# marl/l3embedding

Hardware: AMD Instinct MI355X
Metric: AVC training pairs/sec (1s audio + 224x224 frame) (higher is better)
Workload: dtype f32; 1 GPU; full cnn_L3_melspec2 AVC training step (audio+vision+fusion, fwd+bwd+Adam), batch 64 per GPU, global batch 64, fp32, inputs resident in HBM; global_batch=64, parallelism=dp1, fp32_conv=f4x4

## Files before the change

### include/l3hip.h

```cpp
#ifndef L3HIP_H
#define L3HIP_H

#include <stdint.h>

#ifdef __cplusplus
extern "C" {
#endif

#define L3_OK 0
#define L3_EINVAL (-1)
#define L3_EHIP (-2)
#define L3_ENOMEM (-3)
#define L3_ESTATE (-4)
#define L3_ECOMM (-5)

#define L3_MODEL_CNN_L3_ORIG 0
#define L3_MODEL_TINY_L3 1
#define L3_MODEL_CNN_L3_KAPREDBINPUTBN 2
#define L3_MODEL_CNN_L3_MELSPEC1 3
#define L3_MODEL_CNN_L3_MELSPEC2 4

typedef struct l3_engine l3_engine;

#define L3_DTYPE_F32 0
// ... 178 lines not shown
                           float *mean, float *var, int n, int h, int wd, int cin, int cout, int kh, int kw, int same,
                           int stat_mode);
int l3_op_conv2d_dgrad_bn_bwd(int device, int dtype, const float *dy, const float *w, const float *bn_x, const float *gamma,
                              const float *beta, const float *mean, const float *var, float *dx, float *part, int *nblk,
                              float *dgamma, float *dbeta, int n, int h, int wd, int cin, int cout, int kh, int kw, int same,
                              int relu, int64_t bn_rows);
int l3_op_first_block_bwd(int device, int form, int relu, const float *x, const float *gamma_in, const float *beta_in, const float *w,
                          const float *y, const float *gamma2, const float *beta2, const float *dA, float *mean_in, float *var_in,
                          float *xaug, float *mean2, float *var2, float *scale2, float *shift2, float *dgamma2, float *dbeta2,
                          float *coeffs, float *dY, float *gaug, float *dw, float *dbias, float *dgamma_in, float *dbeta_in, int n,
                          int h, int wd, int c, int cout);
int l3_op_first_conv_grads(int device, const float *gaug, const float *w, const float *gamma, const float *beta, float *dw,
                           float *dgamma, float *dbeta, float *dbias, int taps, int c, int co);
int l3_op_bn_relu_pool2_fwd_xwin(int device, const float *x, const float *gamma, const float *beta, float *p, float *mean,
                                 float *var, float *xwin, int n, int h, int wd, int c, int same, int relu_mode, int x_bf16);
int l3_op_preprocess(int device, const uint8_t *video_u8, int64_t nv, float *video,
                     const int16_t *audio_i16, int64_t na, float *audio);
int l3_op_augment_video(int device, const uint8_t *u8, int n, int h, int w, const l3_augment_params *params,
                        uint8_t *out_u8, float *out_f32);
int l3_op_augment_audio(int device, const int16_t *i16, int n, int t, const double *u, int16_t *out_i16, float *out_f32,
                        double *gains);

typedef struct l3_mlp l3_mlp;
int l3_mlp_create(int device, int D, int C, int batch, float weight_decay, uint64_t seed, l3_mlp **m);
void l3_mlp_destroy(l3_mlp *m);
int64_t l3_mlp_param_count(const l3_mlp *m);
int l3_mlp_set_data(l3_mlp *m, const float *X_train, const int32_t *y_train, int64_t n_train,
                    const float *X_valid, const int32_t *y_valid, int64_t n_valid);
int l3_mlp_epoch(l3_mlp *m, const int32_t *perm, float lr, int64_t t0, double *stats_out);
int l3_mlp_predict(l3_mlp *m, const float *X, int64_t n, float *probs_out);
// ... 195 lines not shown
```

### l3embedding_amd/_lib.py

```python
import ctypes as C
import os

import numpy as np

from . import _build

MODEL_IDS = {
    'cnn_L3_orig': 0,
    'tiny_L3': 1,
    'cnn_L3_kapredbinputbn': 2,
    'cnn_L3_melspec1': 3,
    'cnn_L3_melspec2': 4,
}

FAMILIES = ('conv_fwd', 'conv_dgrad', 'conv_wgrad', 'elementwise', 'frontend', 'head', 'adam')


DTYPES = {'f32': 0, 'fp32': 0, 'float32': 0, 'bf16': 1}
FP32_CONV = {'f4x4': 0, 'f2x2': 1, 'f2x2_bf16x6': 2}
DP_MOVING = {'replicas': 0, 'rank_local': 1}
OP_DTYPES = dict(DTYPES, bf16_stored=2, bf16_stored_out=3)


class L3Config(C.Structure):
# ... 125 lines not shown
    'l3_op_gather_frames': (C.c_int, [C.c_int, C.c_void_p, C.c_int64, C.c_void_p, C.c_int64, C.c_void_p]),
    'l3_op_image_frames': (C.c_int, [C.c_int, C.c_void_p, C.c_int64, C.c_void_p, C.c_int64, C.c_void_p, C.c_void_p]),
    'l3_op_resample': (C.c_int, [C.c_int, C.c_void_p, C.c_int64, C.c_int64, C.c_int64, C.c_void_p, C.c_int64, C.c_int,
                                 C.c_int64, C.c_int64, C.c_void_p]),
    'l3_op_resample_clips': (C.c_int, [C.c_int, C.c_void_p, C.c_int64, C.c_void_p, C.c_int64, C.c_int64, C.c_void_p, C.c_int64,
                                       C.c_int, C.c_int64, C.c_int, C.c_void_p]),
    'l3_op_bn_stats_from_partials': (C.c_int, [C.c_int, C.c_void_p, C.c_int, C.c_int, C.c_void_p, C.c_int64, C.c_float,
                                               C.c_void_p, C.c_void_p]),
    'l3_op_conv2d_fwd_stats': (C.c_int, [C.c_int, C.c_int] + [C.c_void_p] * 5 + [C.POINTER(C.c_int), C.c_void_p, C.c_void_p] +
                               [C.c_int] * 9),
    'l3_op_conv2d_dgrad_bn_bwd': (C.c_int, [C.c_int, C.c_int] + [C.c_void_p] * 9 + [C.POINTER(C.c_int), C.c_void_p, C.c_void_p] +
                                  [C.c_int] * 9 + [C.c_int64]),
    'l3_op_first_block_bwd': (C.c_int, [C.c_int] * 3 + [C.c_void_p] * 24 + [C.c_int] * 5),
    'l3_op_first_conv_grads': (C.c_int, [C.c_int] + [C.c_void_p] * 8 + [C.c_int] * 3),
    'l3_op_bn_relu_pool2_fwd_xwin': (C.c_int, [C.c_int] + [C.c_void_p] * 7 + [C.c_int] * 7),
    'l3_op_preprocess': (C.c_int, [C.c_int, C.c_void_p, C.c_int64, C.c_void_p, C.c_void_p, C.c_int64, C.c_void_p]),
    'l3_op_augment_video': (C.c_int, [C.c_int, C.c_void_p, C.c_int, C.c_int, C.c_int, C.c_void_p, C.c_void_p, C.c_void_p]),
    'l3_op_augment_audio': (C.c_int, [C.c_int, C.c_void_p, C.c_int, C.c_int, C.c_void_p, C.c_void_p, C.c_void_p, C.c_void_p]),
    'l3_mlp_create': (C.c_int, [C.c_int, C.c_int, C.c_int, C.c_int, C.c_float, C.c_uint64, C.POINTER(C.c_void_p)]),
    'l3_mlp_destroy': (None, [C.c_void_p]),
    'l3_mlp_param_count': (C.c_int64, [C.c_void_p]),
    'l3_mlp_set_data': (C.c_int, [C.c_void_p, C.c_void_p, C.c_void_p, C.c_int64, C.c_void_p, C.c_void_p, C.c_int64]),
    'l3_mlp_epoch': (C.c_int, [C.c_void_p, C.c_void_p, C.c_float, C.c_int64, C.POINTER(C.c_double)]),
    'l3_mlp_predict': (C.c_int, [C.c_void_p, C.c_void_p, C.c_int64, C.c_void_p]),
    'l3_mlp_get_weights': (C.c_int, [C.c_void_p, C.c_void_p, C.c_int64]),
    'l3_mlp_set_weights': (C.c_int, [C.c_void_p, C.c_void_p, C.c_int64]),
    'l3_op_mlp_dense_fwd': (C.c_int, [C.c_int, C.c_void_p, C.c_int64, C.c_void_p, C.c_int, C.c_int, C.c_int, C.c_void_p,
                                      C.c_void_p, C.c_int, C.c_void_p]),
    'l3_op_mlp_dense_bwd_x': (C.c_int, [C.c_int, C.c_void_p, C.c_void_p, C.c_void_p, C.c_int, C.c_int, C.c_int, C.c_void_p]),
    'l3_op_mlp_wgrad': (C.c_int, [C.c_int, C.c_void_p, C.c_int64, C.c_void_p, C.c_int, C.c_int, C.c_int, C.c_void_p,
# ... 706 lines not shown
                                      _ptr(var), n, h, wd, c, int(same), int(relu_mode), flags))
    return p, mean, var


def op_bn_relu_pool2_bwd(x, gamma, beta, dp, same, device=0, relu_mode=1, x_bf16=False, out_bf16=False):
    lib = load()
    x, dp = _f32(x), _f32(dp)
    n, h, wd, c = x.shape
    dx = np.empty_like(x)
    dg, db, dbias = (np.empty((c,), np.float32) for _ in range(3))
    check(lib.l3_op_bn_relu_pool2_bwd(device, _ptr(x), _ptr(_f32(gamma)), _ptr(_f32(beta)), _ptr(dp), _ptr(dx),
                                      _ptr(dg), _ptr(db), _ptr(dbias), n, h, wd, c, int(same), int(relu_mode), int(x_bf16) | (4 if out_bf16 else 0)))
    return dx, dg, db, dbias


def _pool_out(h, p, s, same):
    return -(-h // s) if same else (h - p) // s + 1


def op_maxpool_fwd(x, ph, pw, sh, sw, same, device=0):
    lib = load()
    x = _f32(x)
    n, h, wd, c = x.shape
    y = np.empty((n, _pool_out(h, ph, sh, same), _pool_out(wd, pw, sw, same), c), np.float32)
    check(lib.l3_op_maxpool_fwd(device, _ptr(x), _ptr(y), n, h, wd, c, ph, pw, sh, sw, int(same)))
    return y


def op_maxpool_bwd(x, dy, ph, pw, sh, sw, same, device=0):
    lib = load()
# ... 1147 lines not shown
```

### l3embedding_amd/csrc/bn_fused.hip

```cpp
#include "kernels.h"
#include "device_common.h"

namespace l3 {



__device__ __forceinline__ void store_quad(void* base, int64_t q, f32x4 v, int obf) {
    if (obf) {
        bf16x4 h;
        h[0] = (__bf16)v.x; h[1] = (__bf16)v.y; h[2] = (__bf16)v.z; h[3] = (__bf16)v.w;
        __builtin_nontemporal_store(h, reinterpret_cast<bf16x4*>(base) + q);
    } else {
        __builtin_nontemporal_store(v, reinterpret_cast<f32x4*>(base) + q);
    }
}

template <bool XBF>
__device__ __forceinline__ f32x4 load_quad(const void* base, int64_t q) {
    if constexpr (XBF) {
        const u32x2 r = __builtin_nontemporal_load(reinterpret_cast<const u32x2*>(base) + q);
        return f32x4{__uint_as_float(r.x << 16), __uint_as_float(r.x & 0xffff0000u), __uint_as_float(r.y << 16),
                     __uint_as_float(r.y & 0xffff0000u)};
    } else {
        return __builtin_nontemporal_load(reinterpret_cast<const f32x4*>(base) + q);
// ... 563 lines not shown
    const int nb_a = fast_blocks(work_a);
    float* part2 = dbias ? part : nullptr;
    using ApplyFn = void (*)(const void*, const void*, const f32x4*, const f32x4*, const f32x4*, const f32x4*, const f32x4*, void*,
                             float*, int64_t, Pool2Geom, int, int);
    static const ApplyFn apply_fns[8] = {
        bn_bwd_apply_fast_kernel<false, false, false>, bn_bwd_apply_fast_kernel<false, false, true>,
        bn_bwd_apply_fast_kernel<false, true, false>,  bn_bwd_apply_fast_kernel<false, true, true>,
        bn_bwd_apply_fast_kernel<true, false, false>,  bn_bwd_apply_fast_kernel<true, false, true>,
        bn_bwd_apply_fast_kernel<true, true, false>,   bn_bwd_apply_fast_kernel<true, true, true>};
    hipLaunchKernelGGL(apply_fns[variant], dim3(nb_a), dim3(FB), 0, s, xv, dyv, sc4, sh4, reinterpret_cast<const f32x4*>(cA),
                       reinterpret_cast<const f32x4*>(cB), reinterpret_cast<const f32x4*>(cC), (void*)dx, part2, n4, g, relu,
                       dx_bf16);
    if (dbias) launch_fast_final(SumFinal{dbias}, part, nb_a, C, s);
}

}
```

### l3embedding_amd/csrc/elementwise.hip

```cpp
#include <algorithm>

#include "kernels.h"

namespace l3 {

static constexpr int RED_BLOCK = 256;
static constexpr int RED_MAX_BLOCKS = 1024;
static constexpr int SMALLC_MAX = 16;

static inline int red_blocks(int64_t rows, int C) {
    int rows_per_pass = (C % 4 == 0 && C >= 4 && C <= 1024) ? (RED_BLOCK / (C / 4) > 0 ? RED_BLOCK / (C / 4) : 1) : RED_BLOCK;
    int64_t b = (rows + (int64_t)rows_per_pass * 16 - 1) / ((int64_t)rows_per_pass * 16);
    if (b < 1) b = 1;
    if (b > RED_MAX_BLOCKS) b = RED_MAX_BLOCKS;
    return (int)b;
}

size_t colreduce_scratch_floats(int64_t rows, int C) {
    const size_t a = (size_t)red_blocks(rows, C) * 2 * (size_t)(C < 4 ? 4 : C) + 64;
    const size_t b = bn_fast_ok(C) ? bn_fast_scratch_floats(C) : 0;
    return a > b ? a : b;
}

template <class F>
// ... 510 lines not shown
    int arg[4];
    const size_t base = (size_t)n * P * C + cb * 64 + cq * 4;
    gp_scan(x + base, P, C, pg, best, arg);
    gp_merge(sb, sa, pg, cq, best, arg);
    const gp4 d = *reinterpret_cast<const gp4*>(dy + (size_t)n * out_batch_stride + cb * 64 + cq * 4);
    int am[4];
#pragma unroll
    for (int e = 0; e < 4; ++e) am[e] = sa[0][cq * 4 + e];
    for (int p = pg; p < P; p += 16) {
        gp4 o;
#pragma unroll
        for (int e = 0; e < 4; ++e) o[e] = p == am[e] ? d[e] : 0.f;
        *reinterpret_cast<gp4*>(dx + base + (size_t)p * C) = o;
    }
}
static bool is_global_pool(const PoolGeom& g) {
    return g.Ho == 1 && g.Wo == 1 && g.padT == 0 && g.padL == 0 && g.ph == g.H && g.pw == g.W && g.C % 64 == 0 &&
           g.out_batch_stride % 4 == 0;
}

void maxpool_fwd(const float* x, float* y, const PoolGeom& g, hipStream_t s) {
    if (is_global_pool(g)) {
        hipLaunchKernelGGL(global_maxpool_fwd_kernel, dim3(g.N * (g.C / 64)), dim3(256), 0, s, x, y, g.H * g.W, g.C,
                           (int64_t)g.out_batch_stride);
        return;
    }
    const int64_t total = (int64_t)g.N * g.Ho * g.Wo * g.C;
    hipLaunchKernelGGL(maxpool_fwd_kernel, dim3(ew_blocks(total)), dim3(256), 0, s, x, y, g);
}
__global__ __launch_bounds__(256) void maxpool_bwd_kernel(const float* x, const float* dy, float* dx, PoolGeom g) {
    const int64_t total = (int64_t)g.N * g.Ho * g.Wo * g.C;
// ... 395 lines not shown
```

### l3embedding_amd/csrc/engine.hip

```cpp
#include <hip/hip_runtime.h>
#include "knobs.h"

#include <cmath>
#include <cstdio>
#include <cstdlib>
#include <cstring>
#include <map>
#include <string>
#include <vector>

#include "../../include/l3hip.h"
#include "comm.h"
#include "conv_path.h"
#include "featprep.h"
#include "kernels.h"

namespace {

using namespace l3;

static thread_local std::string g_create_error;

constexpr float BN_EPS = 1e-3f;
constexpr float BN_MOMENTUM = 0.99f;
// ... 29 lines not shown
};

enum FirstWgrad { FW_NONE, FW_AUG, FW_AUG_DEFERRED };
struct ConvPlan {
    ConvStorage st;
    ConvFwdPath fwd;
    int stat_mode = 0;
    FirstWgrad aug = FW_NONE;
    ConvWgradPath wgrad;
    bool colsum = false;
    ConvDgradPath dgrad;
    int bwd_bn = -1;
    double fwd_bytes = 0.0, wg_bytes = 0.0, dg_bytes = 0.0;
};
enum BnStats { BS_PARTIALS, BS_FAST, BS_PLAIN, BS_MOVING };
enum BnBwd { BB_BY_FIRST_CONV, BB_FAST_POOLED, BB_FAST, BB_FAST_DEFERRED, BB_PLAIN };
struct BnPlan {
    BnStats stats = BS_MOVING;
    int stat_blocks = 0;
    BnBwd bwd = BB_PLAIN;
    int bwd_blocks = 0;
    double fwd_bytes = 0.0, bwd_bytes = 0.0;
};

struct Op {
    OpKind kind;
    std::string name;
    int in = 0, out = 0;
    int block = 0, bucket = 0;
    int kh = 0, kw = 0, cout = 0;
    bool same = false;
// ... 6 lines not shown
    bool fused_first = false;
    bool defer_apply = false;
    int bn_defer = -1;
    float *xaug = nullptr, *gaug = nullptr;
    ConvGeom ageom{};
    int bn_follow = -1;
    bool need_dx = true;
    int dy_to_bn = -1;
    float* xwin = nullptr;
    int p_gamma = -1, p_beta = -1, p_mmean = -1, p_mvar = -1;
    bool fused_relu = false;
    bool prerelu = false;
    int fuse_pool = -1;
    int bias_param = -1;
    bool fused_into_bn = false;
    bool bias_by_bn = false;
    float *mean = nullptr, *var = nullptr, *scale = nullptr, *shift = nullptr;
    float *biased_mean = nullptr, *biased_var = nullptr;
    PoolGeom pg{};
    ConvPlan cp{};
    BnPlan bp{};
};

struct Tower {
    std::string prefix;
    std::vector<Tensor> t;
    std::vector<Op> ops;
    int nblocks = 0;
    int emb_conv_op = -1;
    bool training = false;
// ... 507 lines not shown
                tw->ops[i + 1].fused_into_bn = true;
            }
        }
    const int first_wg_fuse = knob_int("L3_FIRST_WG_FUSE", 1);
    if (first_wg_fuse)
        for (Tower* tw : {&e->vis, &e->aud})
            for (auto& cv : tw->ops) {
                if (cv.kind != OP_CONV || cv.in_bn < 0 || cv.bn_follow < 0 || !cv.bias_by_bn) continue;
                Op& bn = tw->ops[cv.bn_follow];
                if (bn.kind == OP_BN && bn.fuse_pool < 0 && !bn.prerelu && bn.in == cv.out && bn_fast_ok(cv.cout) &&
                    conv_first_wgrad_ok(cv.ageom)) {
                    bn.defer_apply = true;
                    cv.bn_defer = cv.bn_follow;
                }
            }
    const int pooled_fuse = knob_int("L3_BNBWD_FUSE_POOLED", 1);
    if (bnbwd_fuse && pooled_fuse)
        for (Tower* tw : {&e->vis, &e->aud})
            for (size_t i = 0; i < tw->ops.size(); ++i) {
                Op& cv = tw->ops[i];
                if (cv.kind != OP_CONV || !cv.need_dx || cv.dy_to_bn >= 0) continue;
                for (size_t j = 0; j < i; ++j) {
                    const Op& bn = tw->ops[j];
                    if (bn.kind == OP_BN && bn.fuse_pool >= 0 && tw->ops[bn.fuse_pool].out == cv.in && (bn.fused_relu != bn.prerelu) &&
                        bn_fast_ok(tw->t[bn.in].C))
                        cv.dy_to_bn = (int)j;
                }
            }
    return L3_OK;
}
// ... 333 lines not shown
                y.alias = true;
                if (op.kind == OP_POOL) op.pg.out_batch_stride = D;
            } else if ((op.kind == OP_BN && op.fuse_pool >= 0) || (op.kind == OP_RELU && op.fused_into_bn)) {
                if (op.kind == OP_BN) {
                    bool wanted = false;
                    for (size_t ci = 0; ci < tw.ops.size(); ++ci)
                        if (tw.ops[ci].kind == OP_CONV && tw.ops[ci].dy_to_bn == (int)oi) wanted = true;
                    const Tensor& pl = tw.t[tw.ops[op.fuse_pool].out];
                    if (wanted && (rc = dev_alloc_t(e, &op.xwin, t_floats(pl, tw.t[op.in].d_bf16)))) return rc;
                }
            } else {
                if ((rc = dev_alloc_t(e, &y.d, t_floats(y, y.d_bf16)))) return rc;
                if ((rc = dev_alloc_t(e, &y.g, t_floats(y, y.g_bf16)))) return rc;
            }
            const Tensor& x = tw.t[op.in];
            if (op.kind == OP_CONV) {
                if ((rc = dev_alloc_t(e, &op.wflip, (size_t)e->params[op.p_kernel].numel))) return rc;
                if (conv_wino_floats(op.geom) && (rc = dev_alloc_t(e, &op.wino_uf, conv_wino_floats(op.geom)))) return rc;
                {
                    const size_t sf = (size_t)conv_wino_stat_blocks_max(op.geom) * 2 * op.geom.Cout;
                    if (sf > stat_max) stat_max = sf;
                    const size_t sb = (size_t)conv_bf16_stat_blocks(op.geom) * 2 * op.geom.Cout;
                    if (e->cfg.dtype == L3_DTYPE_BF16 && sb > stat_max) stat_max = sb;
                    const size_t s1 = (size_t)conv_first_stat_blocks(op.geom) * 2 * op.geom.Cout;
                    if (s1 > stat_max) stat_max = s1;
                    const size_t sd = op.dy_to_bn >= 0 ? (size_t)conv_wino_stat_blocks_max(op.dgeom) * 2 * op.dgeom.Cout : 0;
                    if (sd > stat_max) stat_max = sd;
                    const size_t sdb = op.dy_to_bn >= 0 && e->cfg.dtype == L3_DTYPE_BF16
                                           ? (size_t)conv_bf16_stat_blocks(op.dgeom) * 2 * op.dgeom.Cout : 0;
                    if (sdb > stat_max) stat_max = sdb;
// ... 97 lines not shown
        conv_fwd(e->frames, e->wdft, nullptr, e->spec, g, e->stream);
    }
    {
        ProfScope ps(e, F_FRONTEND, f.n_mels ? 2.0 * B * f.n_frames * (double)f.n_freq * f.n_mels : 0.0);
        spec_to_features(e->spec, e->melw, e->mel_start, e->mel_len, e->mel_off, e->aud.t[0].d, B, f, e->stream, e->dft_nyq);
        if (f.db) db_normalize(e->aud.t[0].d, e->smax, B, e->aud.t[0].batch_stride, e->cfg.db_max_scope, e->stream);
    }
    return L3_OK;
}

static inline double act_bytes(const Tensor& t) { return (double)t.numel() * (t.d_bf16 ? 2.0 : 4.0); }
static inline double grad_bytes(const Tensor& t) { return (double)t.numel() * (t.g_bf16 ? 2.0 : 4.0); }

int plan_tower(l3_engine* e, Tower& tw, bool training, int solo) {
    static const int epi_stats = knob_int("L3_EPILOGUE_STATS", 1);
    const bool bf16 = e->cfg.dtype == L3_DTYPE_BF16;
    tw.training = training;
    auto fits = [&](const Op& cv, int blocks, int C) {
        if ((size_t)blocks * 2 * C <= e->stat_max) return true;
        e->err = cv.name + ": " + std::to_string(blocks) + " partial blocks of " + std::to_string(C) + " channels exceed the statistics scratch (" +
                 std::to_string(e->stat_max) + " floats)";
        return false;
    };
    auto defers = [&](const Op& bn) {
        return training && bn.defer_apply && bn.fuse_pool < 0 && bn_fast_ok(tw.t[bn.in].C) && tw.t[bn.in].d_bf16 == tw.t[bn.out].g_bf16;
    };
    for (auto& op : tw.ops) op.bp = BnPlan{};
    for (auto& op : tw.ops) {
        if (op.kind != OP_CONV) continue;
        op.geom.solo = op.dgeom.solo = solo;
        op.geom.dynamic = op.dgeom.dynamic = e->comm != nullptr ? 1 : 0;
        float* ts = solo ? e->w4_tail : nullptr;
        op.geom.tail_scratch = op.dgeom.tail_scratch = ts;
        op.geom.tail_scratch_bytes = op.dgeom.tail_scratch_bytes = ts ? conv_wino4_tail_scratch_bytes() : 0;

        const Tensor &x = tw.t[op.in], &y = tw.t[op.out];
        const double wbytes = (double)e->params[op.p_kernel].numel * 4.0;
        ConvPlan& p = op.cp = ConvPlan{};
        p.st = ConvStorage{bf16, x.d_bf16, y.d_bf16, y.g_bf16, x.g_bf16};
        p.fwd = conv_resolve_fwd(op.geom, p.st, op.wino_uf != nullptr);
        p.fwd_bytes = act_bytes(x) + act_bytes(y) + wbytes;
        const int nblk = conv_fwd_stat_blocks(p.fwd, op.geom);
// ... 25 lines not shown
    }
    for (auto& op : tw.ops) {
        if (op.kind != OP_BN) continue;
        const Tensor &x = tw.t[op.in], &y = tw.t[op.out];
        const Tensor& out = op.fuse_pool >= 0 ? tw.t[tw.ops[op.fuse_pool].out] : y;
        BnPlan& p = op.bp;
        p.stats = !training ? BS_MOVING : p.stat_blocks > 0 ? BS_PARTIALS : op.prerelu || x.d_bf16 ? BS_FAST : BS_PLAIN;
        p.bwd = training && op.fused_first ? BB_BY_FIRST_CONV : !bn_fast_ok(x.C) ? BB_PLAIN : op.fuse_pool >= 0 ? BB_FAST_POOLED
                : defers(op) ? BB_FAST_DEFERRED : BB_FAST;
        p.fwd_bytes = (!training ? 0.0 : p.stat_blocks > 0 ? (double)p.stat_blocks * 2 * x.C * 4 : act_bytes(x)) + act_bytes(x) + act_bytes(out);
        if (p.bwd == BB_BY_FIRST_CONV) p.fwd_bytes += act_bytes(x) + (double)x.rows() * (&op + 1)->ageom.Cin * 4.0;
        if (op.fuse_pool >= 0 && training && op.xwin != nullptr) p.fwd_bytes += (double)out.numel() * (x.d_bf16 ? 2.0 : 4.0);
        p.bwd_bytes = p.bwd == BB_PLAIN ? 2.0 * (act_bytes(x) + grad_bytes(y)) + grad_bytes(x)
                                        : (p.bwd_blocks > 0 ? (double)p.bwd_blocks * 2 * x.C * 4 : act_bytes(x) + grad_bytes(out)) +
                                              (p.bwd == BB_FAST_DEFERRED ? 0.0 : act_bytes(x) + grad_bytes(out) + grad_bytes(x));
    }
    return L3_OK;
}

void tower_forward(l3_engine* e, Tower& tw) {
    const bool training = tw.training;
    for (auto& op : tw.ops) {
        Tensor& x = tw.t[op.in];
        Tensor& y = tw.t[op.out];
        switch (op.kind) {
            case OP_CONV: {
                const ConvPlan& p = op.cp;
                ConvBufs b;
                b.x = x.d, b.w = e->params[op.p_kernel].d, b.bias = e->params[op.p_bias].d, b.y = y.d;
                b.wprep = op.wflip, b.wino_u = op.wino_uf;
// ... 15 lines not shown
                                               op.scale, op.shift, x.rows(), x.C, BN_EPS, op.prerelu ? 1 : 0, e->stream);
                        break;
                    case BS_FAST:
                        bn_stats_fast(x.d, gamma, beta, op.mean, op.var, op.scale, op.shift, e->red_scratch, x.rows(), x.C, BN_EPS,
                                      op.prerelu ? 1 : 0, e->stream, x.d_bf16 ? 1 : 0);
                        break;
                    case BS_PLAIN:
                        bn_stats(x.d, gamma, beta, op.mean, op.var, op.scale, op.shift, e->red_scratch, x.rows(), x.C, BN_EPS, e->stream);
                        break;
                    case BS_MOVING:
                        bn_scale_shift(gamma, beta, e->params[op.p_mmean].d, e->params[op.p_mvar].d, op.scale, op.shift, x.C, BN_EPS,
                                       e->stream);
                        break;
                }
                if (p.bwd == BB_BY_FIRST_CONV) bn_xhat_ones(x.d, op.mean, op.var, BN_EPS, (&op + 1)->xaug, x.rows(), x.C, e->stream);
                if (op.fuse_pool >= 0) {
                    Tensor& pl = tw.t[tw.ops[op.fuse_pool].out];
                    bn_relu_pool2_fwd(x.d, op.scale, op.shift, pl.d, x.N, x.H, x.W, x.C, pl.H, pl.W, pl.batch_stride,
                                      op.prerelu ? 2 : (op.fused_relu ? 1 : 0), e->stream, pl.d_bf16 ? 1 : 0, x.d_bf16 ? 1 : 0,
                                      training ? (void*)op.xwin : nullptr);
                } else if (y.d_bf16 || x.d_bf16) {
                    bn_apply_fast(x.d, op.scale, op.shift, y.d, x.rows(), x.C, op.fused_relu ? 1 : 0, e->stream, y.d_bf16 ? 1 : 0,
                                  x.d_bf16 ? 1 : 0);
                } else {
                    bn_apply(x.d, op.scale, op.shift, y.d, x.rows(), x.C, op.fused_relu ? 1 : 0, e->stream);
                }
                break;
            }
            case OP_RELU: {
                if (op.fused_into_bn) break;
                ProfScope ps(e, F_ELEMWISE, 0.0);
                ps.bytes(act_bytes(x) + act_bytes(y));
                relu_fwd(x.d, y.d, x.numel(), e->stream);
                break;
            }
            case OP_POOL: {
                if (op.fused_into_bn) break;
                ProfScope ps(e, F_ELEMWISE, 0.0);
                ps.bytes(act_bytes(x) + act_bytes(y));
                maxpool_fwd(x.d, y.d, op.pg, e->stream);
                break;
            }
            default: break;
        }
    }
}

BnBwdFuse bn_bwd_fuse(const Tower& tw, const Op& bn) {
    return BnBwdFuse{bn.fuse_pool >= 0 ? bn.xwin : tw.t[bn.in].d, bn.scale, bn.shift, bn.mean, bn.var, BN_EPS, bn.fused_relu ? 1 : 0};
}

void tower_backward_block(l3_engine* e, Tower& tw, int block) {
    const bool training = tw.training;
    for (int oi = (int)tw.ops.size() - 1; oi >= 0; --oi) {
        Op& op = tw.ops[oi];
        if (op.block != block) continue;
        Tensor& x = tw.t[op.in];
        Tensor& y = tw.t[op.out];
        switch (op.kind) {
            case OP_POOL: {
                if (op.fused_into_bn) break;
                ProfScope ps(e, F_ELEMWISE, 0.0);
                ps.bytes(act_bytes(x) + grad_bytes(y) + grad_bytes(x));
                maxpool_bwd(x.d, y.g, x.g, op.pg, e->stream);
                break;
            }
            case OP_RELU: {
                if (op.fused_into_bn) break;
                ProfScope ps(e, F_ELEMWISE, 0.0);
                ps.bytes(act_bytes(y) + grad_bytes(y) + grad_bytes(x));
                relu_bwd(y.d, y.g, x.g, x.numel(), e->stream);
                break;
            }
            case OP_BN: {
                const BnPlan& p = op.bp;
                if (p.bwd == BB_BY_FIRST_CONV) break;
                ProfScope ps(e, F_ELEMWISE, 0.0);
                ps.bytes(p.bwd_bytes);
                const float* mean = training ? op.mean : e->params[op.p_mmean].d;
                const float* var = training ? op.var : e->params[op.p_mvar].d;
                const float* gamma = e->params[op.p_gamma].d;
                float *dgamma = e->params[op.p_gamma].g, *dbeta = e->params[op.p_beta].g;
                if (p.bwd == BB_PLAIN) {
                    bn_bwd(x.d, y.d, y.g, gamma, mean, var, x.g, dgamma, dbeta, e->red_scratch, x.rows(), x.C, BN_EPS, op.fused_relu ? 1 : 0,
                           training ? 1 : 0, e->stream);
                    break;
                }
                const bool pooled = p.bwd == BB_FAST_POOLED, defer = p.bwd == BB_FAST_DEFERRED;
                const Tensor& dy = pooled ? tw.t[tw.ops[op.fuse_pool].out] : y;
                bn_bwd_fast(x.d, op.scale, op.shift, mean, var, gamma, dy.g, pooled ? 1 : 0, x.N, x.H, x.W, x.C, dy.H, dy.W,
                            pooled ? dy.batch_stride : (int64_t)x.H * x.W * x.C, defer ? nullptr : x.g, dgamma, dbeta,
                            defer ? nullptr : op.bias_param >= 0 ? e->params[op.bias_param].g : nullptr, e->red_scratch, BN_EPS,
                            pooled ? (op.prerelu ? 2 : 1) : (op.fused_relu ? 1 : 0), training ? 1 : 0, e->stream, x.g_bf16 ? 1 : 0,
                            x.d_bf16 ? 1 : 0, dy.g_bf16 ? 1 : 0, p.bwd_blocks > 0 ? e->stat_scratch : nullptr, p.bwd_blocks);
                break;
            }
            case OP_CONV: {
                const ConvPlan& p = op.cp;
                const float* w = e->params[op.p_kernel].d;
                if (p.aug != FW_NONE) {
// ... 1661 lines not shown
```

### l3embedding_amd/csrc/kernels.h

```cpp
#pragma once
#include <hip/hip_runtime.h>
#include <stdint.h>

#include <string>
#include <vector>

#include "host_common.h"

struct l3_clipbank;
struct l3_sample;

namespace l3 {

struct ConvGeom {
    int N, H, W, Cin;
    int Ho, Wo, Cout;
    int KH, KW, padT, padL;
    int f2x2 = 0;
    int solo = 0;
    int dynamic = 0;
    float* tail_scratch = nullptr;
    size_t tail_scratch_bytes = 0;
};
size_t conv_wino4_tail_scratch_bytes();
// ... 99 lines not shown
                   float* shift, float* scratch, int64_t rows, int C, float eps, int prerelu, hipStream_t s, int x_bf16 = 0);
void bn_stats_from_partials(const float* part, int nblk, const float* pivot, const float* gamma, const float* beta,
                            float* mean, float* var, float* scale, float* shift, int64_t rows, int C, float eps,
                            int prerelu, hipStream_t s);
void bn_apply_fast(const float* x, const float* scale, const float* shift, float* y, int64_t rows, int C, int relu,
                   hipStream_t s, int out_bf16 = 0, int x_bf16 = 0);
void bn_relu_pool2_fwd(const float* x, const float* scale, const float* shift, float* p, int N, int H, int W, int C,
                       int Ho, int Wo, int64_t out_batch_stride, int mode, hipStream_t s, int out_bf16 = 0, int x_bf16 = 0,
                       void* xwin = nullptr);
void bn_bwd_fast(const float* x, const float* scale, const float* shift, const float* mean, const float* var,
                 const float* gamma, const float* dy, int pooled, int N, int H, int W, int C, int Ho, int Wo,
                 int64_t dy_batch_stride, float* dx, float* dgamma, float* dbeta, float* dbias, float* scratch,
                 float eps, int relu, int training, hipStream_t s, int dx_bf16 = 0, int x_bf16 = 0, int dy_bf16 = 0,
                 const float* ready_part = nullptr, int ready_blocks = 0);
const float* bn_bwd_fast_coeffs(const float* scratch, int C);

void relu_fwd(const float* x, float* y, int64_t n, hipStream_t s);
void relu_bwd(const float* y, const float* dy, float* dx, int64_t n, hipStream_t s);

struct PoolGeom {
    int N, H, W, C, Ho, Wo, ph, pw, sh, sw, padT, padL;
    int64_t out_batch_stride;
};
void maxpool_fwd(const float* x, float* y, const PoolGeom& g, hipStream_t s);
void maxpool_bwd(const float* x, const float* dy, float* dx, const PoolGeom& g, hipStream_t s);

void preprocess_video(const uint8_t* u8, float* out, int64_t n, hipStream_t s);
void preprocess_audio(const int16_t* pcm, float* out, int64_t n, hipStream_t s);
void labels_onehot(const int32_t* lab, float* out, int64_t n, hipStream_t s);

struct AugmentParams {
    int32_t start_x, start_y, flip, sat_first;
    float saturation, brightness;
};
constexpr int AUG_CROP = 224;
void augment_video(const uint8_t* u8, int N, int H, int W, const AugmentParams* params, uint8_t* out_u8, float* out_f32,
                   hipStream_t s);
void augment_audio(const int16_t* pcm, int N, int T, const double* u, int16_t* out_i16, float* out_f32, double* gains,
// ... 175 lines not shown
```

### l3embedding_amd/csrc/ops.hip

```cpp
#include <hip/hip_runtime.h>

#include <cstring>
#include <string>
#include <vector>

#include "../../include/l3hip.h"
#include "conv_path.h"
#include "kernels.h"
#include "knobs.h"
#include "mlp.h"
#include "vggish.h"

namespace {
using namespace l3;

struct Scope {
    DeviceBufs bufs;
    hipStream_t s = nullptr;
    bool ok = true;
    explicit Scope(int device) : ok(device_ok(device)) {}
    ~Scope() { (void)hipDeviceSynchronize(); }
    template <class T>
    T* alloc(size_t count) {
        T* p = bufs.alloc<T>(count);
// ... 894 lines not shown
    l3_engine* e = nullptr;
    int rc = l3_create(&cfg, 1, &e);
    if (rc) return rc;
    rc = l3_upload_batch(e, nullptr, audio, nullptr);
    if (!rc) rc = l3_step_forward(e, 0);
    int64_t numel = 0;
    if (!rc) rc = l3_activation_numel(e, "audio_model/frontend", &numel);
    if (!rc) rc = l3_get_activation(e, "audio_model/frontend", out, numel);
    l3_destroy(e);
    return rc;
}

}

namespace {
int mlp_op_check(const char* name, int device, bool ptrs_ok, int rows, int K, int N, const int32_t* idx, int64_t n_x) {
    if (!ptrs_ok || rows <= 0 || K <= 0 || N <= 0 || n_x < 0) {
        set_op_error(std::string(name) + ": NULL pointer or non-positive size");
        return L3_EINVAL;
    }
    if (!idx && n_x < rows) {
        set_op_error(std::string(name) + ": fewer rows in x than `rows`");
        return L3_EINVAL;
    }
    for (int i = 0; idx && i < rows; ++i)
        if (idx[i] < 0 || idx[i] >= n_x) {
            set_op_error(std::string(name) + ": idx[" + std::to_string(i) + "] outside [0, n_x)");
            return L3_EINVAL;
        }
    if (!device_ok(device)) {
// ... 487 lines not shown
```

Before: 2049 pairs/s.

## Fuse final BatchNorm+ReLU with global max pool in tower forward and backward

```diff
diff --git a/include/l3hip.h b/include/l3hip.h
--- a/include/l3hip.h
+++ b/include/l3hip.h
@@ -216,6 +216,10 @@
                            float *dgamma, float *dbeta, float *dbias, int taps, int c, int co);
 int l3_op_bn_relu_pool2_fwd_xwin(int device, const float *x, const float *gamma, const float *beta, float *p, float *mean,
                                  float *var, float *xwin, int n, int h, int wd, int c, int same, int relu_mode, int x_bf16);
+int l3_op_bn_relu_gpool_fwd(int device, const float *x, const float *gamma, const float *beta, float *p, int32_t *arg,
+                            float *mean, float *var, int n, int h, int wd, int c);
+int l3_op_bn_relu_gpool_bwd(int device, const float *x, const float *gamma, const float *beta, const float *dp, float *dx,
+                            float *dgamma, float *dbeta, float *dbias, int n, int h, int wd, int c);
 int l3_op_preprocess(int device, const uint8_t *video_u8, int64_t nv, float *video,
                      const int16_t *audio_i16, int64_t na, float *audio);
 int l3_op_augment_video(int device, const uint8_t *u8, int n, int h, int w, const l3_augment_params *params,
diff --git a/l3embedding_amd/_lib.py b/l3embedding_amd/_lib.py
--- a/l3embedding_amd/_lib.py
+++ b/l3embedding_amd/_lib.py
@@ -163,6 +163,8 @@
     'l3_op_first_block_bwd': (C.c_int, [C.c_int] * 3 + [C.c_void_p] * 24 + [C.c_int] * 5),
     'l3_op_first_conv_grads': (C.c_int, [C.c_int] + [C.c_void_p] * 8 + [C.c_int] * 3),
     'l3_op_bn_relu_pool2_fwd_xwin': (C.c_int, [C.c_int] + [C.c_void_p] * 7 + [C.c_int] * 7),
+    'l3_op_bn_relu_gpool_fwd': (C.c_int, [C.c_int] + [C.c_void_p] * 7 + [C.c_int] * 4),
+    'l3_op_bn_relu_gpool_bwd': (C.c_int, [C.c_int] + [C.c_void_p] * 8 + [C.c_int] * 4),
     'l3_op_preprocess': (C.c_int, [C.c_int, C.c_void_p, C.c_int64, C.c_void_p, C.c_void_p, C.c_int64, C.c_void_p]),
     'l3_op_augment_video': (C.c_int, [C.c_int, C.c_void_p, C.c_int, C.c_int, C.c_int, C.c_void_p, C.c_void_p, C.c_void_p]),
     'l3_op_augment_audio': (C.c_int, [C.c_int, C.c_void_p, C.c_int, C.c_int, C.c_void_p, C.c_void_p, C.c_void_p, C.c_void_p]),
@@ -899,6 +901,29 @@
     return dx, dg, db, dbias
 
 
+def op_bn_relu_gpool_fwd(x, gamma, beta, device=0):
+    lib = load()
+    x = _f32(x)
+    n, h, wd, c = x.shape
+    p, arg = np.empty((n, c), np.float32), np.empty((n, c), np.int32)
+    mean, var = np.empty((c,), np.float32), np.empty((c,), np.float32)
+    check(lib.l3_op_bn_relu_gpool_fwd(device, _ptr(x), _ptr(_f32(gamma)), _ptr(_f32(beta)), _ptr(p), _ptr(arg), _ptr(mean), _ptr(var),
+                                      n, h, wd, c))
+    return p, arg, mean, var
+
+
+def op_bn_relu_gpool_bwd(x, gamma, beta, dp, device=0):
+    lib = load()
+    x, dp = _f32(x), _f32(dp)
+    n, h, wd, c = x.shape
+    assert dp.shape == (n, c)
+    dx = np.empty_like(x)
+    dg, db, dbias = (np.empty((c,), np.float32) for _ in range(3))
+    check(lib.l3_op_bn_relu_gpool_bwd(device, _ptr(x), _ptr(_f32(gamma)), _ptr(_f32(beta)), _ptr(dp), _ptr(dx), _ptr(dg), _ptr(db),
+                                      _ptr(dbias), n, h, wd, c))
+    return dx, dg, db, dbias
+
+
 def _pool_out(h, p, s, same):
     return -(-h // s) if same else (h - p) // s + 1
 
diff --git a/l3embedding_amd/csrc/bn_fused.hip b/l3embedding_amd/csrc/bn_fused.hip
--- a/l3embedding_amd/csrc/bn_fused.hip
+++ b/l3embedding_amd/csrc/bn_fused.hip
@@ -601,4 +601,163 @@
     if (dbias) launch_fast_final(SumFinal{dbias}, part, nb_a, C, s);
 }
 
-}
+static constexpr int GP_G = 16;
+static constexpr int GP_U = 8;
+
+bool bn_relu_gpool_ok(int N, int H, int W, int C) {
+    return bn_fast_ok(C) && C % 64 == 0 && N >= 1 && H >= 1 && W >= 1 && (int64_t)H * W < ((int64_t)1 << 30) &&
+           (int64_t)N * (C / 64) < ((int64_t)1 << 31);
+}
+
+__global__ __launch_bounds__(256) void bn_relu_gpool_fwd_kernel(const float* __restrict__ x, const float* __restrict__ scale,
+                                                                const float* __restrict__ shift, float* __restrict__ out,
+                                                                int* __restrict__ arg, int P, int C, int64_t out_batch_stride) {
+    __shared__ float sb[GP_G][64];
+    __shared__ int sa[GP_G][64];
+    const int cb = blockIdx.x % (C / 64), n = blockIdx.x / (C / 64);
+    const int cq = threadIdx.x & 15, pg = threadIdx.x >> 4;
+    const int c0 = cb * 64 + cq * 4;
+    const f32x4 sc = *reinterpret_cast<const f32x4*>(scale + c0), sh = *reinterpret_cast<const f32x4*>(shift + c0);
+    const f32x4* xb = reinterpret_cast<const f32x4*>(x + (size_t)n * P * C + c0);
+    const size_t C4 = (size_t)(C / 4);
+    float best[4];
+    int am[4];
+#pragma unroll
+    for (int e = 0; e < 4; ++e) {
+        best[e] = -INFINITY;
+        am[e] = 0x7fffffff;
+    }
+    for (int p0 = pg; p0 < P; p0 += GP_G * GP_U) {
+        f32x4 v[GP_U];
+#pragma unroll
+        for (int u = 0; u < GP_U; ++u)
+            if (p0 + u * GP_G < P) v[u] = __builtin_nontemporal_load(xb + (size_t)(p0 + u * GP_G) * C4);
+#pragma unroll
+        for (int u = 0; u < GP_U; ++u) {
+            const int p = p0 + u * GP_G;
+            if (p < P) {
+                const f32x4 r = relu4(bn_pre(v[u], sc, sh));
+#pragma unroll
+                for (int e = 0; e < 4; ++e)
+                    if (r[e] > best[e]) {
+                        best[e] = r[e];
+                        am[e] = p;
+                    }
+            }
+        }
+    }
+#pragma unroll
+    for (int e = 0; e < 4; ++e) {
+        sb[pg][cq * 4 + e] = best[e];
+        sa[pg][cq * 4 + e] = am[e];
+    }
+    __syncthreads();
+    if (threadIdx.x < 64) {
+        float b = sb[0][threadIdx.x];
+        int a = sa[0][threadIdx.x];
+        for (int k = 1; k < GP_G; ++k) {
+            const float vb = sb[k][threadIdx.x];
+            const int va = sa[k][threadIdx.x];
+            if (vb > b || (vb == b && va < a)) {
+                b = vb;
+                a = va;
+            }
+        }
+        out[(size_t)n * out_batch_stride + cb * 64 + threadIdx.x] = b;
+        arg[(size_t)n * C + cb * 64 + threadIdx.x] = a;
+    }
+}
+
+void bn_relu_gpool_fwd(const float* x, const float* scale, const float* shift, float* out, int* arg, int N, int H, int W, int C,
+                       int64_t out_batch_stride, hipStream_t s) {
+    hipLaunchKernelGGL(bn_relu_gpool_fwd_kernel, dim3(N * (C / 64)), dim3(256), 0, s, x, scale, shift, out, arg, H * W, C,
+                       out_batch_stride);
+}
+
+__global__ __launch_bounds__(FB) void bn_gpool_bwd_reduce_kernel(const float* __restrict__ x, const float* __restrict__ dp,
+                                                                 const int* __restrict__ arg, const float* __restrict__ scale,
+                                                                 const float* __restrict__ shift, const float* __restrict__ mean,
+                                                                 const float* __restrict__ var, float* __restrict__ part, int N,
+                                                                 int P, int C, int64_t dp_batch_stride, int npb, float eps) {
+    const int n0 = blockIdx.x * npb, n1 = n0 + npb < N ? n0 + npb : N;
+    for (int c = threadIdx.x; c < C; c += FB) {
+        const float sc = scale[c], sh = shift[c], mu = mean[c], rs = rsqrtf(var[c] + eps);
+        float a0 = 0.f, a1 = 0.f;
+        for (int n = n0; n < n1; ++n) {
+            const int a = arg[(size_t)n * C + c];
+            if ((unsigned)a < (unsigned)P) {
+                const float xv = x[((size_t)n * P + a) * C + c];
+                const float d = fmaf(xv, sc, sh) > 0.f ? dp[(size_t)n * dp_batch_stride + c] : 0.f;
+                a0 += d;
+                a1 += d * ((xv - mu) * rs);
+            }
+        }
+        part[((size_t)blockIdx.x * 2 + 0) * C + c] = a0;
+        part[((size_t)blockIdx.x * 2 + 1) * C + c] = a1;
+    }
+}
+
+__global__ __launch_bounds__(FB) void bn_gpool_bwd_apply_kernel(const float* __restrict__ x, const float* __restrict__ dp,
+                                                                const int* __restrict__ arg, const f32x4* scale, const f32x4* shift,
+                                                                const f32x4* cA, const f32x4* cB, const f32x4* cC,
+                                                                float* __restrict__ dx, float* part, int P, int C4,
+                                                                int64_t dp_bs4, int tiles_per_n, int64_t tiles) {
+    constexpr int U = 4, K = 2;
+    const int c4 = (int)threadIdx.x % C4, r = (int)threadIdx.x / C4, rpi = FB / C4;
+    const f32x4 sc = scale[c4], sh = shift[c4], A = cA[c4], B = cB[c4], Cc = cC[c4];
+    f32x4 a0 = {0.f, 0.f, 0.f, 0.f};
+    for (int64_t t = blockIdx.x; t < tiles; t += gridDim.x) {
+        const int n = (int)(t / tiles_per_n);
+        const int pt = (int)(t % tiles_per_n) * (rpi * U * K);
+        const i32x4 am = reinterpret_cast<const i32x4*>(arg)[(int64_t)n * C4 + c4];
+        const f32x4 d = reinterpret_cast<const f32x4*>(dp)[(int64_t)n * dp_bs4 + c4];
+        const int64_t row0 = (int64_t)n * P;
+#pragma unroll
+        for (int k = 0; k < K; ++k) {
+            const int p0 = pt + k * U * rpi + r;
+            f32x4 v[U];
+#pragma unroll
+            for (int u = 0; u < U; ++u)
+                if (p0 + u * rpi < P) v[u] = load_quad<false>(x, (row0 + p0 + u * rpi) * C4 + c4);
+#pragma unroll
+            for (int u = 0; u < U; ++u) {
+                const int p = p0 + u * rpi;
+                if (p < P) {
+                    const f32x4 pre = bn_pre(v[u], sc, sh);
+                    f32x4 dz;
+                    dz.x = p == am.x && pre.x > 0.f ? d.x : 0.f; dz.y = p == am.y && pre.y > 0.f ? d.y : 0.f;
+                    dz.z = p == am.z && pre.z > 0.f ? d.z : 0.f; dz.w = p == am.w && pre.w > 0.f ? d.w : 0.f;
+                    const f32x4 o = A * dz + (B * v[u] + Cc);
+                    store_quad(dx, (row0 + p) * C4 + c4, o, 0);
+                    a0 += o;
+                }
+            }
+        }
+    }
+    if (part != nullptr) block_write_partials(a0, a0, part, C4);
+}
+
+void bn_relu_gpool_bwd(const float* x, const float* scale, const float* shift, const float* mean, const float* var,
+                       const float* gamma, const float* dp, const int* arg, int N, int H, int W, int C, int64_t dp_batch_stride,
+                       float* dx, float* dgamma, float* dbeta, float* dbias, float* scratch, float eps, hipStream_t s) {
+    const int P = H * W, C4 = C / 4;
+    float* part = scratch;
+    float* cA = scratch + (size_t)FAST_MAX_BLOCKS * 2 * C;
+    float* cB = cA + C;
+    float* cC = cB + C;
+    const int npb = (N + FAST_MAX_BLOCKS - 1) / FAST_MAX_BLOCKS;
+    const int nb_r = (N + npb - 1) / npb;
+    hipLaunchKernelGGL(bn_gpool_bwd_reduce_kernel, dim3(nb_r), dim3(FB), 0, s, x, dp, arg, scale, shift, mean, var, part, N, P, C,
+                       dp_batch_stride, npb, eps);
+    launch_fast_final(BwdFinal{gamma, mean, var, dgamma, dbeta, cA, cB, cC, 1.0 / ((double)N * P), eps, 1}, part, nb_r, C, s);
+    const int tile_px = (FB / C4) * 8;
+    const int tiles_per_n = (P + tile_px - 1) / tile_px;
+    const int64_t tiles = (int64_t)N * tiles_per_n;
+    const int nb_a = (int)(tiles < FAST_MAX_BLOCKS ? tiles : FAST_MAX_BLOCKS);
+    hipLaunchKernelGGL(bn_gpool_bwd_apply_kernel, dim3(nb_a), dim3(FB), 0, s, x, dp, arg, reinterpret_cast<const f32x4*>(scale),
+                       reinterpret_cast<const f32x4*>(shift), reinterpret_cast<const f32x4*>(cA), reinterpret_cast<const f32x4*>(cB),
+                       reinterpret_cast<const f32x4*>(cC), dx, dbias ? part : nullptr, P, C4, dp_batch_stride / 4, tiles_per_n, tiles);
+    if (dbias) launch_fast_final(SumFinal{dbias}, part, nb_a, C, s);
+}
+
+}
diff --git a/l3embedding_amd/csrc/elementwise.hip b/l3embedding_amd/csrc/elementwise.hip
--- a/l3embedding_amd/csrc/elementwise.hip
+++ b/l3embedding_amd/csrc/elementwise.hip
@@ -548,7 +548,7 @@
         *reinterpret_cast<gp4*>(dx + base + (size_t)p * C) = o;
     }
 }
-static bool is_global_pool(const PoolGeom& g) {
+bool is_global_pool(const PoolGeom& g) {
     return g.Ho == 1 && g.Wo == 1 && g.padT == 0 && g.padL == 0 && g.ph == g.H && g.pw == g.W && g.C % 64 == 0 &&
            g.out_batch_stride % 4 == 0;
 }
diff --git a/l3embedding_amd/csrc/engine.hip b/l3embedding_amd/csrc/engine.hip
--- a/l3embedding_amd/csrc/engine.hip
+++ b/l3embedding_amd/csrc/engine.hip
@@ -67,7 +67,7 @@
     double fwd_bytes = 0.0, wg_bytes = 0.0, dg_bytes = 0.0;
 };
 enum BnStats { BS_PARTIALS, BS_FAST, BS_PLAIN, BS_MOVING };
-enum BnBwd { BB_BY_FIRST_CONV, BB_FAST_POOLED, BB_FAST, BB_FAST_DEFERRED, BB_PLAIN };
+enum BnBwd { BB_BY_FIRST_CONV, BB_FAST_POOLED, BB_FAST, BB_FAST_DEFERRED, BB_PLAIN, BB_FAST_GPOOL };
 struct BnPlan {
     BnStats stats = BS_MOVING;
     int stat_blocks = 0;
@@ -104,6 +104,9 @@
     int fuse_pool = -1;
     int bias_param = -1;
     bool fused_into_bn = false;
+    int gpool = -1;
+    int* garg = nullptr;
+    bool pass_by_bn = false;
     bool bias_by_bn = false;
     float *mean = nullptr, *var = nullptr, *scale = nullptr, *shift = nullptr;
     float *biased_mean = nullptr, *biased_var = nullptr;
@@ -641,6 +644,16 @@
                     cv.bn_defer = cv.bn_follow;
                 }
             }
+    for (Tower* tw : {&e->vis, &e->aud})
+        if (tw->ops.size() >= 2) {
+            const size_t i = tw->ops.size() - 2;
+            Op& bn = tw->ops[i];
+            const Op& pl = tw->ops[i + 1];
+            const Tensor& x = tw->t[bn.in];
+            if (bn.kind == OP_BN && bn.fused_relu && !bn.prerelu && bn.fuse_pool < 0 && !bn.fused_first && !bn.defer_apply &&
+                pl.kind == OP_POOL && pl.in == bn.out && is_global_pool(pl.pg) && bn_relu_gpool_ok(x.N, x.H, x.W, x.C))
+                bn.gpool = (int)i + 1;
+        }
     const int pooled_fuse = knob_int("L3_BNBWD_FUSE_POOLED", 1);
     if (bnbwd_fuse && pooled_fuse)
         for (Tower* tw : {&e->vis, &e->aud})
@@ -1004,6 +1017,7 @@
                 if ((rc = dev_alloc_t(e, &y.g, t_floats(y, y.g_bf16)))) return rc;
             }
             const Tensor& x = tw.t[op.in];
+            if (op.kind == OP_BN && op.gpool >= 0 && (rc = dev_alloc_t(e, &op.garg, (size_t)x.N * x.C))) return rc;
             if (op.kind == OP_CONV) {
                 if ((rc = dev_alloc_t(e, &op.wflip, (size_t)e->params[op.p_kernel].numel))) return rc;
                 if (conv_wino_floats(op.geom) && (rc = dev_alloc_t(e, &op.wino_uf, conv_wino_floats(op.geom)))) return rc;
@@ -1131,6 +1145,7 @@
 
 int plan_tower(l3_engine* e, Tower& tw, bool training, int solo) {
     static const int epi_stats = knob_int("L3_EPILOGUE_STATS", 1);
+    const int tower_end = knob_int("L3_TOWER_END_FUSE", 1);
     const bool bf16 = e->cfg.dtype == L3_DTYPE_BF16;
     tw.training = training;
     auto fits = [&](const Op& cv, int blocks, int C) {
@@ -1142,7 +1157,10 @@
     auto defers = [&](const Op& bn) {
         return training && bn.defer_apply && bn.fuse_pool < 0 && bn_fast_ok(tw.t[bn.in].C) && tw.t[bn.in].d_bf16 == tw.t[bn.out].g_bf16;
     };
-    for (auto& op : tw.ops) op.bp = BnPlan{};
+    for (auto& op : tw.ops) {
+        op.bp = BnPlan{};
+        op.pass_by_bn = false;
+    }
     for (auto& op : tw.ops) {
         if (op.kind != OP_CONV) continue;
         op.geom.solo = op.dgeom.solo = solo;
@@ -1198,6 +1216,17 @@
         p.bwd_bytes = p.bwd == BB_PLAIN ? 2.0 * (act_bytes(x) + grad_bytes(y)) + grad_bytes(x)
                                         : (p.bwd_blocks > 0 ? (double)p.bwd_blocks * 2 * x.C * 4 : act_bytes(x) + grad_bytes(out)) +
                                               (p.bwd == BB_FAST_DEFERRED ? 0.0 : act_bytes(x) + grad_bytes(out) + grad_bytes(x));
+        if (!tower_end || !training || bf16 || p.bwd != BB_FAST || op.gpool < 0 || op.garg == nullptr) continue;
+        Op& pl = tw.ops[op.gpool];
+        const Tensor& po = tw.t[pl.out];
+        if (!is_global_pool(pl.pg) || x.d_bf16 || x.g_bf16 || po.d_bf16 || po.g_bf16 || x.batch_stride != (int64_t)x.H * x.W * x.C ||
+            po.batch_stride != pl.pg.out_batch_stride)
+            continue;
+        p.bwd = BB_FAST_GPOOL;
+        pl.pass_by_bn = true;
+        const double nc = (double)x.N * x.C * 4.0;
+        p.fwd_bytes = (p.stat_blocks > 0 ? (double)p.stat_blocks * 2 * x.C * 4 : act_bytes(x)) + act_bytes(x) + 2.0 * nc;
+        p.bwd_bytes = 3.0 * nc + act_bytes(x) + 2.0 * nc + grad_bytes(x);
     }
     return L3_OK;
 }
@@ -1243,7 +1272,10 @@
                         break;
                 }
                 if (p.bwd == BB_BY_FIRST_CONV) bn_xhat_ones(x.d, op.mean, op.var, BN_EPS, (&op + 1)->xaug, x.rows(), x.C, e->stream);
-                if (op.fuse_pool >= 0) {
+                if (p.bwd == BB_FAST_GPOOL) {
+                    Tensor& pl = tw.t[tw.ops[op.gpool].out];
+                    bn_relu_gpool_fwd(x.d, op.scale, op.shift, pl.d, op.garg, x.N, x.H, x.W, x.C, pl.batch_stride, e->stream);
+                } else if (op.fuse_pool >= 0) {
                     Tensor& pl = tw.t[tw.ops[op.fuse_pool].out];
                     bn_relu_pool2_fwd(x.d, op.scale, op.shift, pl.d, x.N, x.H, x.W, x.C, pl.H, pl.W, pl.batch_stride,
                                       op.prerelu ? 2 : (op.fused_relu ? 1 : 0), e->stream, pl.d_bf16 ? 1 : 0, x.d_bf16 ? 1 : 0,
@@ -1264,7 +1296,7 @@
                 break;
             }
             case OP_POOL: {
-                if (op.fused_into_bn) break;
+                if (op.fused_into_bn || op.pass_by_bn) break;
                 ProfScope ps(e, F_ELEMWISE, 0.0);
                 ps.bytes(act_bytes(x) + act_bytes(y));
                 maxpool_fwd(x.d, y.d, op.pg, e->stream);
@@ -1288,7 +1320,7 @@
         Tensor& y = tw.t[op.out];
         switch (op.kind) {
             case OP_POOL: {
-                if (op.fused_into_bn) break;
+                if (op.fused_into_bn || op.pass_by_bn) break;
                 ProfScope ps(e, F_ELEMWISE, 0.0);
                 ps.bytes(act_bytes(x) + grad_bytes(y) + grad_bytes(x));
                 maxpool_bwd(x.d, y.g, x.g, op.pg, e->stream);
@@ -1313,6 +1345,13 @@
                 if (p.bwd == BB_PLAIN) {
                     bn_bwd(x.d, y.d, y.g, gamma, mean, var, x.g, dgamma, dbeta, e->red_scratch, x.rows(), x.C, BN_EPS, op.fused_relu ? 1 : 0,
                            training ? 1 : 0, e->stream);
+                    break;
+                }
+                if (p.bwd == BB_FAST_GPOOL) {
+                    const Tensor& pl = tw.t[tw.ops[op.gpool].out];
+                    bn_relu_gpool_bwd(x.d, op.scale, op.shift, mean, var, gamma, pl.g, op.garg, x.N, x.H, x.W, x.C, pl.batch_stride, x.g,
+                                      dgamma, dbeta, op.bias_param >= 0 ? e->params[op.bias_param].g : nullptr, e->red_scratch, BN_EPS,
+                                      e->stream);
                     break;
                 }
                 const bool pooled = p.bwd == BB_FAST_POOLED, defer = p.bwd == BB_FAST_DEFERRED;
diff --git a/l3embedding_amd/csrc/kernels.h b/l3embedding_amd/csrc/kernels.h
--- a/l3embedding_amd/csrc/kernels.h
+++ b/l3embedding_amd/csrc/kernels.h
@@ -137,6 +137,12 @@
                  float eps, int relu, int training, hipStream_t s, int dx_bf16 = 0, int x_bf16 = 0, int dy_bf16 = 0,
                  const float* ready_part = nullptr, int ready_blocks = 0);
 const float* bn_bwd_fast_coeffs(const float* scratch, int C);
+bool bn_relu_gpool_ok(int N, int H, int W, int C);
+void bn_relu_gpool_fwd(const float* x, const float* scale, const float* shift, float* out, int* arg, int N, int H, int W, int C,
+                       int64_t out_batch_stride, hipStream_t s);
+void bn_relu_gpool_bwd(const float* x, const float* scale, const float* shift, const float* mean, const float* var,
+                       const float* gamma, const float* dp, const int* arg, int N, int H, int W, int C, int64_t dp_batch_stride,
+                       float* dx, float* dgamma, float* dbeta, float* dbias, float* scratch, float eps, hipStream_t s);
 
 void relu_fwd(const float* x, float* y, int64_t n, hipStream_t s);
 void relu_bwd(const float* y, const float* dy, float* dx, int64_t n, hipStream_t s);
@@ -145,6 +151,7 @@
     int N, H, W, C, Ho, Wo, ph, pw, sh, sw, padT, padL;
     int64_t out_batch_stride;
 };
+bool is_global_pool(const PoolGeom& g);
 void maxpool_fwd(const float* x, float* y, const PoolGeom& g, hipStream_t s);
 void maxpool_bwd(const float* x, const float* dy, float* dx, const PoolGeom& g, hipStream_t s);
 
diff --git a/l3embedding_amd/csrc/ops.hip b/l3embedding_amd/csrc/ops.hip
--- a/l3embedding_amd/csrc/ops.hip
+++ b/l3embedding_amd/csrc/ops.hip
@@ -932,6 +932,90 @@
 }
 
 namespace {
+int gpool_common(const char* name, int device, const float* x, const float* gamma, const float* beta, const float* dp, float* p,
+                 int32_t* arg, float* mean, float* var, float* dx, float* dgamma, float* dbeta, float* dbias, int n, int h, int wd,
+                 int c) {
+    if (!x || !gamma || !beta || (dp ? !dx || !dgamma || !dbeta || !dbias : !p || !arg || !mean || !var)) {
+        set_op_error(std::string(name) + ": NULL pointer");
+        return L3_EINVAL;
+    }
+    const PoolGeom g = n >= 1 && h >= 1 && wd >= 1 && c >= 1 ? make_pool(n, h, wd, c, h, wd, h, wd, 0) : PoolGeom{};
+    if (n < 1 || h < 1 || wd < 1 || c < 1 || !is_global_pool(g) || !bn_relu_gpool_ok(n, h, wd, c)) {
+        set_op_error(std::string(name) + ": an engine would run the separate BatchNorm and pool kernels here (c a power of two in [64, 1024])");
+        return L3_EINVAL;
+    }
+    Scope sc(device);
+    if (!sc.ok) return L3_EHIP;
+    const int64_t rows = (int64_t)n * h * wd;
+    const size_t nx = (size_t)rows * c, np_ = (size_t)n * c, co = (size_t)c, guard = 1024;
+    const uint32_t nan_bits = 0x7fc00000u;
+    float sentinel = -12345.f;
+    uint32_t sentinel_bits;
+    memcpy(&sentinel_bits, &sentinel, sizeof sentinel_bits);
+    auto fresh = [&](size_t count) {
+        float* q = sc.alloc<float>(count + guard);
+        if (q && (hipMemsetD32(reinterpret_cast<hipDeviceptr_t>(q), (int)nan_bits, count) != hipSuccess ||
+                  hipMemsetD32(reinterpret_cast<hipDeviceptr_t>(q + count), (int)sentinel_bits, guard) != hipSuccess))
+            sc.ok = false;
+        return q;
+    };
+    bool guards_ok = true;
+    auto take = [&](void* host, const float* dev, size_t count, const char* what) {
+        std::vector<float> gd(guard);
+        sc.get(gd.data(), dev + count, guard);
+        for (size_t i = 0; sc.ok && guards_ok && i < guard; ++i)
+            if (memcmp(&gd[i], &sentinel, sizeof sentinel) != 0) {
+                set_op_error(std::string(name) + ": word " + std::to_string(i) + " of the guard behind " + what + " changed");
+                guards_ok = false;
+            }
+        sc.get(reinterpret_cast<float*>(host), dev, count);
+    };
+    float* d_x = sc.put(x, nx);
+    float *d_g = sc.put(gamma, co), *d_b = sc.put(beta, co);
+    float *d_m = sc.alloc<float>(co), *d_v = sc.alloc<float>(co), *d_sc = sc.alloc<float>(co), *d_sh = sc.alloc<float>(co);
+    float* d_p = fresh(np_);
+    float* d_arg = fresh(np_);
+    size_t red = colreduce_scratch_floats(rows, c);
+    if (bn_fast_scratch_floats(c) > red) red = bn_fast_scratch_floats(c);
+    float* d_red = sc.alloc<float>(red);
+    if (!sc.ok) return L3_ENOMEM;
+    bn_stats(d_x, d_g, d_b, d_m, d_v, d_sc, d_sh, d_red, rows, c, 1e-3f, sc.s);
+    bn_relu_gpool_fwd(d_x, d_sc, d_sh, d_p, reinterpret_cast<int*>(d_arg), n, h, wd, c, g.out_batch_stride, sc.s);
+    if (!dp) {
+        take(p, d_p, np_, "the pooled values");
+        take(arg, d_arg, np_, "the winner indices");
+        sc.get(mean, d_m, co);
+        sc.get(var, d_v, co);
+    } else {
+        float* d_dp = sc.put(dp, np_);
+        float* d_dx = fresh(nx);
+        float *d_dg = fresh(co), *d_db = fresh(co), *d_dbias = fresh(co);
+        if (!sc.ok) return L3_ENOMEM;
+        bn_relu_gpool_bwd(d_x, d_sc, d_sh, d_m, d_v, d_g, d_dp, reinterpret_cast<const int*>(d_arg), n, h, wd, c, g.out_batch_stride,
+                          d_dx, d_dg, d_db, d_dbias, d_red, 1e-3f, sc.s);
+        take(dx, d_dx, nx, "dx");
+        take(dgamma, d_dg, co, "dgamma");
+        take(dbeta, d_db, co, "dbeta");
+        take(dbias, d_dbias, co, "dbias");
+    }
+    const int rc = sc.status();
+    return rc ? rc : guards_ok ? L3_OK : L3_EINVAL;
+}
+}
+
+extern "C" int l3_op_bn_relu_gpool_fwd(int device, const float* x, const float* gamma, const float* beta, float* p, int32_t* arg,
+                                       float* mean, float* var, int n, int h, int wd, int c) {
+    return gpool_common("l3_op_bn_relu_gpool_fwd", device, x, gamma, beta, nullptr, p, arg, mean, var, nullptr, nullptr, nullptr,
+                        nullptr, n, h, wd, c);
+}
+
+extern "C" int l3_op_bn_relu_gpool_bwd(int device, const float* x, const float* gamma, const float* beta, const float* dp, float* dx,
+                                       float* dgamma, float* dbeta, float* dbias, int n, int h, int wd, int c) {
+    return gpool_common("l3_op_bn_relu_gpool_bwd", device, x, gamma, beta, dp, nullptr, nullptr, nullptr, nullptr, dx, dgamma, dbeta,
+                        dbias, n, h, wd, c);
+}
+
+namespace {
 int mlp_op_check(const char* name, int device, bool ptrs_ok, int rows, int K, int N, const int32_t* idx, int64_t n_x) {
     if (!ptrs_ok || rows <= 0 || K <= 0 || N <= 0 || n_x < 0) {
         set_op_error(std::string(name) + ": NULL pointer or non-positive size");
```

Result: no change. 2064 pairs/s (median of 6 runs) (+0.7%).
